# awikner/SPEEDY-ML-1

Hardware: AMD Instinct MI355X
Metric: hybrid timesteps/sec, T30L8 + 1152x6k-node reservoirs; 1/2/4/8-GPU scaling (higher is better)
Workload: dtype f64

## Files before the change

### include/speedy_ml.h

```cpp
#ifndef SPEEDY_ML_H
#define SPEEDY_ML_H

#include <stddef.h>
#include <stdint.h>

#ifdef __cplusplus
extern "C" {
#endif

#define SML_OK 0
#define SML_ERR_ARG (-1)
#define SML_ERR_HIP (-2)
#define SML_ERR_NOMEM (-3)
#define SML_ERR_STATE (-4)
#define SML_ERR_IO (-5)
#define SML_ERR_FORMAT (-6)

#define SML_F32 1
#define SML_F64 2

#define SML_MX 31
#define SML_NX 32
#define SML_MX2 62
#define SML_IX 96
// ... 85 lines not shown
int sml_nc_read_region(const char *path, int64_t *dims, float *win, float *wout, int *rows, int *cols, float *vals,
                       float *mean, float *std);
int sml_nc_write_region(const char *path, int n, int ninp, int nout, int ncs_plus_n, int k, const float *win,
                        const float *wout, const int *rows, const int *cols, const float *vals, const float *mean,
                        const float *std);

typedef struct sml_dynamics sml_dynamics;

int sml_dyn_create(double radius, sml_dynamics **out);
int sml_dyn_destroy(sml_dynamics *d);
int sml_dyn_impint(sml_dynamics *d, double dt, double alph);
int sml_dyn_set_forcing(sml_dynamics *d, const double *phis, const double *tcorh, const double *qcorh);
int sml_dyn_set_state(sml_dynamics *d, const double *vor, const double *div, const double *t, const double *ps,
                      const double *tr);
int sml_dyn_get_state(sml_dynamics *d, double *vor, double *div, double *t, double *ps, double *tr);
int sml_dyn_get_phi(sml_dynamics *d, double *phi);
int sml_dyn_get_tendencies(sml_dynamics *d, double *tend);
int sml_dyn_state_device(sml_dynamics *d, double **d_state, double **d_phys);
int sml_dyn_step(sml_dynamics *d, int j1, int j2, double dt, double alph, double rob, double wil,
                 const double *d_phys, void *stream);
int sml_dyn_leapfrog(sml_dynamics *d, int nsteps, double dt, double alph, double rob, double wil,
                     const double *d_phys, void *stream);
int sml_dyn_window(sml_dynamics *d, int nleap, double delt, double alph, double rob, double wil, void *stream);
int sml_dyn_from_grid(sml_dynamics *d, const double *d_grid4d, const double *d_logp, double *d_minmax,
                      void *stream);
int sml_dyn_to_grid(sml_dynamics *d, double *d_grid4d, double *d_logp, void *stream);
int sml_dyn_is_safe(const double *minmax);
int sml_dyn_run_model(sml_dynamics *d, const double *d_grid4d, const double *d_logp, int nleap, double delt,
                      double alph, double rob, double wil, double *d_fc4d, double *d_fc2d, void *stream);
int sml_dyn_last_safe(sml_dynamics *d, int *safe, double *minmax);
int sml_dyn_set_check_cus(sml_dynamics *d, int first_cu, int num_cus);
int sml_dyn_set_check_timeout(sml_dynamics *d, int64_t microseconds);
int sml_dyn_set_fused(sml_dynamics *d, int fused);
int sml_dyn_check_stream(const sml_dynamics *d, void **stream);
int sml_dyn_from_grid_host(sml_dynamics *d, const double *grid4d, const double *logp, double *minmax, int *safe);
int sml_dyn_to_grid_host(sml_dynamics *d, double *grid4d, double *logp);
int sml_dyn_step_host(sml_dynamics *d, int j1, int j2, double dt, double alph, double rob, double wil,
                      const double *phys);

int sml_dyn_set_physics(sml_dynamics *d, const double *bc);
int sml_dyn_set_hybrid_sst(sml_dynamics *d, const double *d_sst_grid, double sst_bias, void *stream);
int sml_dyn_set_sea_ice(sml_dynamics *d, const double *sice, const double *tice);
int sml_dyn_get_sea_ice(sml_dynamics *d, double *sice, double *tice);
int sml_dyn_get_physics(sml_dynamics *d, double *bc);
int sml_dyn_get_forcing(sml_dynamics *d, double *phis, double *tcorh, double *qcorh);
int sml_dyn_set_surface(sml_dynamics *d, const double *surface);
int sml_dyn_set_climatology(sml_dynamics *d, const double *clim);
int sml_dyn_fordate(sml_dynamics *d, int iyear, int imonth, int iday, void *stream);
int sml_dyn_fordate_ex(sml_dynamics *d, int iyear, int imonth, int iday, int force, void *stream);
int sml_dyn_fordate_count(const sml_dynamics *d, int *count);
int sml_dyn_set_clock(sml_dynamics *d, int istep, int lradsw);
int sml_dyn_get_clock(const sml_dynamics *d, int *istep, int *lradsw);
int sml_dyn_set_rad_state(sml_dynamics *d, const double *rad);
int sml_dyn_get_rad_state(sml_dynamics *d, double *rad);
int sml_dyn_phypar(sml_dynamics *d, const double *d_ug1, const double *d_vg1, const double *d_tg1,
                   const double *d_qg1, const double *d_phig1, const double *d_pslg1, int lradsw, double *d_tend,
                   void *stream);
int sml_dyn_phypar_host(sml_dynamics *d, const double *ug1, const double *vg1, const double *tg1, const double *qg1,
                        const double *phig1, const double *pslg1, int lradsw, double *tend);
int sml_dyn_sol_oz(const sml_dynamics *d, double tyear, double *fields5);
int sml_phys_sflset(const double *phi0, double *forog);

typedef struct sml_train sml_train;
int sml_train_create(int nlocal, const int *naug, int nout, sml_train **out);
int sml_train_destroy(sml_train *t);
int sml_train_reset(sml_train *t, void *stream);
// ... 88 lines not shown
```

### speedy-ml-1_amd/csrc/sml_dynamics.hip

```cpp
#include <hip/hip_runtime.h>

#include <cmath>
#include <cstddef>
#include <cstdlib>
#include <cstring>
#include <new>
#include <vector>

#include "sml_dynamics_tables.hpp"
#include "sml_fft.hpp"
#include "sml_fft_wa96.hpp"
#include "sml_physics.hpp"
#include "sml_physics_pair.hpp"
#include "sml_spectral_internal.hpp"
#include "sml_timeline.hpp"

SML_TL_DEFINE(dynamics)

using namespace sml;

namespace {

constexpr int kSF = kMX2 * kNX;
constexpr int kGF = kIX * kIL;
// ... 52 lines not shown
    unsigned chk_count = 0;
    bool chk_counted = false;
    double *h_mm = nullptr;
    hipEvent_t ev_mm = nullptr;
    bool mm_issued = false;
    const double *mm_last = nullptr;
    bool impint_done = false;
    PhysTables ptab;
    PhysTables *d_ptab = nullptr;
    double *d_pbc = nullptr, *d_rad = nullptr, *d_pio = nullptr;
    bool phys_on = false;
    double *d_sst_cpl = nullptr, *d_sice = nullptr, *d_tice = nullptr;
    const double *hyb_sst = nullptr;
    double hyb_bias = 0.0;
    double *d_surf = nullptr, *d_clim = nullptr, *d_ford = nullptr;
    bool surf_on = false, clim_on = false;
    long long ford_gen = 1, ford_done = 0;
    int ford_date[2] = {0, 0};
    int ford_count = 0;
    bool fused = true;
    bool nograph = false;
    bool lradsw = true;
    int istep = 1;
    hipStream_t cap_stream = nullptr;
    struct Replay {
        hipGraphExec_t exec = nullptr;
        double key[4] = {0, 0, 0, 0};
        const double *phys = nullptr;
        const DynTables *tab = nullptr;
        bool phys_on = false;
    } replay[2];
    struct WindowReplay {
        hipGraphExec_t exec = nullptr;
        double key[8] = {0, 0, 0, 0, 0, 0, 0, 0};
        DynTables *tab[3] = {nullptr, nullptr, nullptr};
        bool has_exit = false;
        const void *exit_key[16] = {};
    };
    static constexpr int kReplayWays = 4;
    WindowReplay wreplay[4][kReplayWays];
    int wreplay_next[4] = {0, 0, 0, 0};
    uint64_t *exit_store = nullptr;
    uint64_t exit_store_value = 0;
    uint64_t *d_xa = nullptr;
    bool entry_graph = true;
    bool serialized = false;
    uint64_t *d_go = nullptr;
    uint64_t go_count = 0;
    const uint64_t *go_src_next = nullptr;
    uint64_t *go_dst_next = nullptr;
    double *io_exit = nullptr;
};

namespace {

__device__ inline void uvspec_at(const double *vor, const double *div, const DynTables *T, int m, int n, double *uc,
                                 double *vc) {
    const double ux = T->uvdx[n][m];
    double zp[2], zc[2];
    zp[1] = ux * vor[ci(0, m, n)];
    zp[0] = -ux * vor[ci(1, m, n)];
    zc[1] = ux * div[ci(0, m, n)];
    zc[0] = -ux * div[ci(1, m, n)];
#pragma unroll
    for (int p = 0; p < 2; ++p) {
        double a, b;
        if (n == 0) {
            a = zc[p] - T->uvdyp[0][m] * vor[ci(p, m, 1)];
            b = zp[p] + T->uvdyp[0][m] * div[ci(p, m, 1)];
        } else if (n == kNX - 1) {
            a = T->uvdym[n][m] * vor[ci(p, m, kNTRUN1 - 1)];
            b = -T->uvdym[n][m] * div[ci(p, m, kNTRUN1 - 1)];
        } else {
            b = -T->uvdym[n][m] * div[ci(p, m, n - 1)] + T->uvdyp[n][m] * div[ci(p, m, n + 1)] + zp[p];
            a = T->uvdym[n][m] * vor[ci(p, m, n - 1)] - T->uvdyp[n][m] * vor[ci(p, m, n + 1)] + zc[p];
        }
        uc[ci(p, m, n)] = a;
        vc[ci(p, m, n)] = b;
// ... 1264 lines not shown
    if (mn >= kMN) return;
    const int k = blockIdx.y;
    const int m = mn % kMX, n = mn / kMX;
    const double trf = T->trfilt[n][m];
#pragma unroll
    for (int p = 0; p < 2; ++p) {
        const int c = ci(p, m, n);
        double vo, dv;
        vds_at(S + (size_t)k * kSF, S + (size_t)(kKX + k) * kSF, T, m, n, p, &vo, &dv);
        st[kOffVor + (size_t)k * kSF + c] = vo * trf;
        st[kOffDiv + (size_t)k * kSF + c] = dv * trf;
        st[kOffT + (size_t)k * kSF + c] = S[(size_t)(2 * kKX + k) * kSF + c] * trf;
        st[kOffTr + (size_t)k * kSF + c] = S[(size_t)(3 * kKX + k) * kSF + c] * trf;
        if (k == 0) st[kOffPs + c] = S[(size_t)(4 * kKX) * kSF + c] * trf;
    }
}

__global__ void k_io_prep(const double *__restrict__ st, double *__restrict__ sin_, const DynTables *__restrict__ T) {
    const int mn = blockIdx.x * blockDim.x + threadIdx.x;
    if (mn >= kMN) return;
    const int k = blockIdx.y;
    const int m = mn % kMX, n = mn / kMX;
    const double *vor = st + kOffVor + (size_t)k * kSF, *div = st + kOffDiv + (size_t)k * kSF;
    uvspec_at(vor, div, T, m, n, sin_ + (size_t)k * kSF, sin_ + (size_t)(kKX + k) * kSF);
#pragma unroll
    for (int p = 0; p < 2; ++p) {
        const int c = ci(p, m, n);
        sin_[(size_t)(2 * kKX + k) * kSF + c] = st[kOffT + (size_t)k * kSF + c];
        sin_[(size_t)(3 * kKX + k) * kSF + c] = st[kOffTr + (size_t)k * kSF + c];
        if (k == 0) sin_[(size_t)(4 * kKX) * kSF + c] = st[kOffPs + c];
    }
}

__global__ __launch_bounds__(kSpecThreads) void k_io_entry(const double *__restrict__ vio,
                                                           const double *__restrict__ pfl,
                                                           const double *__restrict__ wt, double *__restrict__ state,
                                                           double *__restrict__ sm, double *__restrict__ chk,
                                                           const double *__restrict__ phis,
                                                           const double *__restrict__ tabm,
                                                           const double *__restrict__ pinv, double *__restrict__ varm,
                                                           int n1, int nin, uint64_t *__restrict__ xa, uint64_t xa0,
                                                           uint64_t xa1) {
    SML_TL_SCOPE(sml::tl::kIoEntry);
    if (xa && blockIdx.x == 0 && threadIdx.x == 0) {
        xa[0] = xa0;
        xa[1] = xa1;
    }
    __shared__ double S[kNIo * kCW];
    __shared__ double Sst[kSM];
    __shared__ double In[kNInvMax * kCW];
    __shared__ double Fm[kCW];
    constexpr int RT = (kTabMDoubles / 2 + kSpecThreads - 1) / kSpecThreads;
    __shared__ double V[2 * RT * kSpecThreads];
    const int m = blockIdx.x, tid = threadIdx.x;
    const int wave = tid >> 6, l = tid & 63, r = l & 15, kk = l >> 4;
    constexpr int kSI = kSM / kSpecThreads;
    static_assert(kSM % kSpecThreads == 0 && kSI == 10, "slice staging: ten rows of the block");
    double s2[kSI / 2];
#pragma unroll
    for (int q = 1; q < kSI; q += 2) {
        const int cc = tid % kCW, k = tid / kCW, var = q / 2;
        const int c = ci(cc & 1, m, cc >> 1);
        double v = 0.0;
        if (var < 4) {
            const size_t off = var == 0 ? kOffVor : var == 1 ? kOffDiv : var == 2 ? kOffT : kOffTr;
            v = state[off + ((size_t)kKX + k) * kSF + c];
        } else if (k == 0) {
            v = state[kOffPs + (size_t)kSF + c];
        }
        s2[q / 2] = v;
    }
    const double phis_m = tid < kCW ? phis[ci(tid & 1, m, tid >> 1)] : 0.0;
    static_assert(2 * RT * kSpecThreads - kTabMDoubles <= kTabMPad, "TabM staging");
    double2 rt[RT];
    {
        const double2 *t = reinterpret_cast<const double2 *>(tabm + (size_t)m * kTabMDoubles) + tid;
#pragma unroll
        for (int q = 0; q < RT; ++q) rt[q] = t[q * kSpecThreads];
    }
    const bool spw = wave < (kNIo + 7) / 8;
    const int f0 = wave * 8, fa = f0 + (r >> 1);
    const bool ok = spw && fa < kNIo;
    double vn[kIY / 4], vs[kIY / 4], wv[kIY / 4], bS[kIY / 4], bD[kIY / 4];
    if (spw) {
        const double *vr = vio + (size_t)(ok ? fa : 0) * kVarmField + 2 * m + (r & 1);
        const double2 *pl = reinterpret_cast<const double2 *>(pfl) + (size_t)m * (kIY / 4) * 64 + l;
#pragma unroll
        for (int s = 0; s < kIY / 4; ++s) {
            const int j = 4 * s + kk;
            vn[s] = vr[(kIL - 1 - j) * kMX2];
            vs[s] = vr[j * kMX2];
            wv[s] = wt[j];
            const double2 b = pl[s * 64];
            bS[s] = b.x;
            bD[s] = b.y;
        }
    }
    const GridyB gb = gridy_operands(pinv, m);
    __builtin_amdgcn_sched_barrier(0);
#pragma unroll
    for (int q = 0; q < RT; ++q) reinterpret_cast<double2 *>(V)[tid + q * kSpecThreads] = rt[q];
#pragma unroll
    for (int q = 1; q < kSI; q += 2) Sst[tid + kSpecThreads * q] = s2[q / 2];
    if (tid < kCW) Fm[tid] = phis_m;
    if (spw) {
        d4 accS = {0, 0, 0, 0}, accD = accS;
#pragma unroll
        for (int s = 0; s < kIY / 4; ++s) {
            double aS = 0.0, aD = 0.0;
            if (ok) {
                aS = (vn[s] + vs[s]) * wv[s];
                aD = (vn[s] - vs[s]) * wv[s];
            }
            accS = MFMA64(aS, bS[s], accS);
            accD = MFMA64(aD, bD[s], accD);
        }
#pragma unroll
        for (int q = 0; q < 4; ++q) {
            const int row = kk + 4 * q;
            const int f = f0 + (row >> 1);
            if (f >= kNIo) continue;
            S[f * kCW + 2 * (2 * r) + (row & 1)] = accS[q];
            S[f * kCW + 2 * (2 * r + 1) + (row & 1)] = accD[q];
        }
    }
    __syncthreads();
    const LTab tb{reinterpret_cast<const TabM *>(V)};
    const int cc = tid & (kCW - 1), k = tid / kCW, n = cc >> 1, p = cc & 1, c = ci(p, m, n);
    {
        auto fl = [&](int f) { return [=](int pp, int nn) { return S[f * kCW + 2 * nn + pp]; }; };
        const double trf = tb.trfilt_n(n);
        double vo, dv;
        vds_gen(fl(k), fl(kKX + k), tb, n, p, &vo, &dv);
        const double v0 = vo * trf, v1 = dv * trf, v2 = S[(2 * kKX + k) * kCW + cc] * trf,
                     v3 = S[(3 * kKX + k) * kCW + cc] * trf;
        Sst[smi(0, 1, k, cc)] = v0;
        Sst[smi(1, 1, k, cc)] = v1;
        Sst[smi(2, 1, k, cc)] = v2;
        Sst[smi(3, 1, k, cc)] = v3;
        state[kOffVor + (size_t)k * kSF + c] = v0;
        state[kOffDiv + (size_t)k * kSF + c] = v1;
        state[kOffT + (size_t)k * kSF + c] = v2;
        state[kOffTr + (size_t)k * kSF + c] = v3;
        if (k == 0) {
            const double v4 = S[(4 * kKX) * kCW + cc] * trf;
            Sst[smi(4, 1, 0, cc)] = v4;
            state[kOffPs + c] = v4;
        } else {
            Sst[smi(4, 1, k, cc)] = 0.0;
        }
    }
    __syncthreads();
    {
        double a, b;
        uvspec_sel(Sst, tb, 1, k, n, p, &a, &b);
        chk[(size_t)k * kSF + c] = a;
        chk[(size_t)(kKX + k) * kSF + c] = b;
        chk[(size_t)(2 * kKX + k) * kSF + c] = Sst[smi(2, 1, k, cc)];
        chk[(size_t)(3 * kKX + k) * kSF + c] = Sst[smi(3, 1, k, cc)];
        if (k == 0) chk[(size_t)(4 * kKX) * kSF + c] = Sst[smi(4, 1, 0, cc)];
    }
    {
        static_assert(kSM / 2 % kSpecThreads == 0, "slice rows");
        constexpr int R = kSM / 2 / kSpecThreads;
        double2 *dst = reinterpret_cast<double2 *>(sm + (size_t)m * kSM) + tid;
        const double2 *src = reinterpret_cast<const double2 *>(Sst) + tid;
        double2 v[R];
#pragma unroll
        for (int q = 0; q < R; ++q) v[q] = src[q * kSpecThreads];
#pragma unroll
        for (int q = 0; q < R; ++q) dst[q * kSpecThreads] = v[q];
    }
    inv_inputs(Sst, In, Fm, tb, m, 1, n1, nin);
    __syncthreads();
    gridy_m(In, gb, varm, m, nin);
}

__device__ inline double nmin(double a, double b) { return (a != a || b != b) ? __builtin_nan("") : (b < a ? b : a); }
__device__ inline double nmax(double a, double b) { return (a != a || b != b) ? __builtin_nan("") : (b > a ? b : a); }

__global__ void k_flag_store_value(uint64_t *flag, uint64_t v) {
    SML_TL_SCOPE(sml::tl::kExitStore);
    if (threadIdx.x == 0) __hip_atomic_store(flag, v, __ATOMIC_RELAXED, __HIP_MEMORY_SCOPE_AGENT);
}
__global__ void k_set_xa(uint64_t *xa, uint64_t v0, uint64_t v1, uint64_t v2, uint64_t v3) {
    if (threadIdx.x == 0) {
        xa[0] = v0;
        xa[1] = v1;
        xa[2] = v2;
        xa[3] = v3;
    }
}

__global__ void k_check_go(const uint64_t *go, uint64_t want, unsigned *late, unsigned late_value, long long timeout) {
    if (threadIdx.x != 0) return;
    const long long t0 = wall_clock64();
    while (__hip_atomic_load(go, __ATOMIC_RELAXED, __HIP_MEMORY_SCOPE_AGENT) < want) {
        __builtin_amdgcn_s_sleep(2);
        if (wall_clock64() - t0 > timeout) {
            __hip_atomic_store(late, late_value, __ATOMIC_RELAXED, __HIP_MEMORY_SCOPE_SYSTEM);
            break;
        }
    }
    __builtin_amdgcn_fence(__ATOMIC_ACQUIRE, "agent");
}

__global__ void k_flag_store(uint64_t *flag, const uint64_t *xa) {
    SML_TL_SCOPE(sml::tl::kExitStore);
// ... 421 lines not shown
                              void *stream) {
    SML_REQUIRE(d && nleap >= 0 && delt > 0.0, "bad argument");
    return window_impl(d, nleap, delt, alph, rob, wil, stream, false);
}

namespace {
int window_impl(sml_dynamics *d, int nleap, double delt, double alph, double rob, double wil, void *stream,
                bool prepared, const ExitSpec *exit) {
    const double dts[3] = {0.5 * delt, delt, 2.0 * delt};
    DynTables *tab[3];
    for (int i = 0; i < 3; ++i) {
        if (int rc = sml_dyn_impint(d, dts[i], alph)) return rc;
        tab[i] = d->d_tab;
    }
    const bool entry = d->lradsw;
    if (d->nograph) {
        hipStream_t st = (hipStream_t)stream;
        d->d_tab = tab[0];
        d->io_exit = prepared ? d->d_varm : nullptr;
        int rc = launch_step(d, 1, 1, dts[0], alph, rob, wil, nullptr, entry, st, prepared, 2);
        d->d_tab = tab[1];
        if (!rc) rc = launch_step(d, 1, 2, dts[1], alph, rob, wil, nullptr, entry, st, true, nleap > 0 ? 2 : 0);
        d->d_tab = tab[2];
        for (int i = 0; i < nleap && !rc; ++i)
            rc = launch_step(d, 2, 2, dts[2], alph, rob, wil, nullptr, (1 + i) % kNstrad == 1, st, true,
                             i + 1 < nleap ? 2 : 0);
        d->io_exit = nullptr;
        if (rc) return rc;
        d->istep = 1 + nleap;
        if (nleap > 0) d->lradsw = (nleap % kNstrad == 1);
        return SML_OK;
    }
    const int cls = (entry ? 1 : 0) + (prepared ? 2 : 0);
    const double key[8] = {(double)nleap, delt,  alph, rob, wil, d->phys_on ? 1.0 : 0.0, d->fused ? 1.0 : 0.0,
                           prepared ? 2.0 : 1.0};
    const void *exit_key[16] = {};
    if (exit) {
        const EntrySpec *en = exit->entry;
        const void *k[16] = {exit->varm,   exit->fc4,     exit->fc2,    exit->ex.mm,
                             exit->ex.in4, exit->ex.inlp, exit->ex.cnt, (const void *)(intptr_t)exit->ex.timeout,
                             exit->store,  en ? (const void *)1 : nullptr,
                             en ? en->w.flag : nullptr, en ? en->w.late : nullptr, en ? en->w.sig : nullptr,
                             en ? (const void *)(intptr_t)en->w.timeout : nullptr, en ? en->w.vptr : nullptr,
                             en ? en->go : nullptr};
        std::memcpy(exit_key, k, sizeof k);
    }
    auto same = [&](const sml_dynamics::WindowReplay &w) {
        return w.exec && w.has_exit == (exit != nullptr) &&
               (!exit || std::memcmp(exit_key, w.exit_key, sizeof exit_key) == 0) &&
               std::memcmp(key, w.key, sizeof key) == 0 && std::memcmp(tab, w.tab, sizeof tab) == 0;
    };
    sml_dynamics::WindowReplay *hit = nullptr;
    for (auto &w : d->wreplay[cls])
        if (same(w)) hit = &w;
    if (!hit) {
        hit = &d->wreplay[cls][d->wreplay_next[cls]];
        d->wreplay_next[cls] = (d->wreplay_next[cls] + 1) % sml_dynamics::kReplayWays;
    }
    sml_dynamics::WindowReplay &r = *hit;
    if (!same(r)) {
        if (r.exec) {
            SML_HIP(hipGraphExecDestroy(r.exec));
            r.exec = nullptr;
        }
        r.has_exit = false;
        if (!d->cap_stream) SML_HIP(hipStreamCreateWithFlags(&d->cap_stream, hipStreamNonBlocking));
        hipGraph_t g = nullptr;
        SML_HIP(hipStreamBeginCapture(d->cap_stream, hipStreamCaptureModeThreadLocal));
// ... 8 lines not shown
        d->io_exit = prepared ? d->d_varm : nullptr;
        if (!rc) rc = launch_step(d, 1, 1, dts[0], alph, rob, wil, nullptr, entry, d->cap_stream, prepared, 2);
        d->go_src_next = nullptr;
        d->go_dst_next = nullptr;
        d->d_tab = tab[1];
        if (!rc) rc = launch_step(d, 1, 2, dts[1], alph, rob, wil, nullptr, entry, d->cap_stream, true, nleap > 0 ? 2 : 0);
        d->d_tab = tab[2];
        for (int i = 0; i < nleap && !rc; ++i)
            rc = launch_step(d, 2, 2, dts[2], alph, rob, wil, nullptr, (1 + i) % kNstrad == 1, d->cap_stream, true,
                             i + 1 < nleap ? 2 : 0);
        if (!rc && exit) {
            rc = spectral_gridx_run_model_exit(d->sp, exit->varm, exit->fc4, exit->fc2, kNIoWind, exit->ex,
                                               d->cap_stream);
            if (!rc && exit->store) {
                hipLaunchKernelGGL(k_flag_store, dim3(1), dim3(64), 0, d->cap_stream, exit->store, exit->ex.xa);
                if (hipGetLastError() != hipSuccess) rc = fail(SML_ERR_HIP, "k_flag_store capture");
            }
        }
        hipError_t e = hipStreamEndCapture(d->cap_stream, &g);
        d->io_exit = nullptr;
        if (rc) {
            if (g) (void)hipGraphDestroy(g);
            return rc;
        }
        if (e != hipSuccess) return fail(SML_ERR_HIP, "sml_dyn_window capture: %s", hipGetErrorString(e));
        e = hipGraphInstantiate(&r.exec, g, nullptr, nullptr, 0);
        if (e != hipSuccess) {
            (void)hipGraphDestroy(g);
            r.exec = nullptr;
            return fail(SML_ERR_HIP, "sml_dyn_window instantiate: %s", hipGetErrorString(e));
        }
        (void)hipGraphDestroy(g);
        r.has_exit = exit != nullptr;
        std::memcpy(r.exit_key, exit_key, sizeof exit_key);
        std::memcpy(r.key, key, sizeof key);
        std::memcpy(r.tab, tab, sizeof tab);
    }
    SML_HIP(hipGraphLaunch(r.exec, (hipStream_t)stream));
    d->d_tab = tab[2];
    d->istep = 1 + nleap;
    if (nleap > 0) d->lradsw = (nleap % kNstrad == 1);
    return SML_OK;
}
}

extern "C" int sml_dyn_set_clock(sml_dynamics *d, int istep, int lradsw) {
    SML_REQUIRE(d, "null context");
    d->istep = istep;
    d->lradsw = lradsw != 0;
    return SML_OK;
}

extern "C" int sml_dyn_get_clock(const sml_dynamics *d, int *istep, int *lradsw) {
    SML_REQUIRE(d, "null context");
    if (istep) *istep = d->istep;
    if (lradsw) *lradsw = d->lradsw ? 1 : 0;
    return SML_OK;
}

namespace {
__global__ void k_hybrid_sst(const double *__restrict__ cpl, const double *__restrict__ hyb,
                             const double *__restrict__ sice, const double *__restrict__ tice, double bias,
                             double *__restrict__ sst_am) {
#pragma clang fp contract(off)
    const int p = blockIdx.x * blockDim.x + threadIdx.x;
    if (p >= kNGP) return;
    double s = cpl[p];
    if (hyb) {
        const double diff = s - hyb[p];
        if (diff < 6.0) s = hyb[p];
        s = s + bias;
// ... 320 lines not shown
    if (int rc = spectral_gridx_range(d->sp, cv, cg, kNIo, 0, kNIoWind, cst)) return rc;
    double *mm = d_minmax ? d_minmax : d->d_minmax;
    const bool counted = cst != st && !d_minmax;
    hipLaunchKernelGGL(k_io_minmax, dim3(4), dim3(1024), 0, cst, cg, mm, counted ? d->d_chk_cnt : nullptr,
                       go ? d->d_chk_late : nullptr, 4u * (d->chk_count + 1));
    SML_HIP(hipGetLastError());
    if (counted) ++d->chk_count;
    d->chk_counted = counted;
    d->mm_last = mm;
    d->mm_issued = false;
    if (cst != st) {
        if (!d->h_mm) {
            SML_HIP(hipHostMalloc((void **)&d->h_mm, 8 * sizeof(double), hipHostMallocDefault));
            SML_HIP(hipEventCreateWithFlags(&d->ev_mm, hipEventDisableTiming));
        }
        SML_HIP(hipMemcpyAsync(d->h_mm, mm, 8 * sizeof(double), hipMemcpyDeviceToHost, cst));
        SML_HIP(hipEventRecord(d->ev_mm, cst));
        d->mm_issued = true;
        SML_HIP(hipEventRecord(d->ev_chk, cst));
        d->chk_pending = true;
        if (d_minmax) {
            SML_HIP(hipStreamWaitEvent(st, d->ev_chk, 0));
            d->chk_pending = false;
        }
    }
    return SML_OK;
}

int launch_entry(sml_dynamics *d, const double *d_grid4d, const double *d_logp, HopWait w, hipStream_t st,
                 uint64_t *xa, uint64_t xa0, uint64_t xa1) {
    if (int rc = spectral_specx_io(d->sp, d_grid4d, d_logp, d->d_vfm, kNIoWind, st, w)) return rc;
    const SpectralDev sd = spectral_dev(d->sp);
    const bool phys = d->phys_on;
    hipLaunchKernelGGL(k_io_entry, dim3(kMX), dim3(kSpecThreads), 0, st, d->d_vfm, d->d_pfl, sd.wt, d->d_state,
                       sm_buf(d, 0), d->d_chk, d->d_phis,
                       d->d_tabm + (size_t)(d->d_tab - d->d_tabs) * kMX * kTabMDoubles, sd.pinv, d->d_varm,
                       phys ? kNInv1P : kNInv1, phys ? kNInvP : kNInv, xa, xa0, xa1);
    SML_HIP(hipGetLastError());
    return SML_OK;
}
}

extern "C" int sml_dyn_from_grid(sml_dynamics *d, const double *d_grid4d, const double *d_logp, double *d_minmax,
                                 void *stream) {
    SML_REQUIRE(d && d_grid4d && d_logp, "null argument");
    hipStream_t st = (hipStream_t)stream;
    const DynTables *T = d->d_tab;
    if (d->chk_pending) {
        SML_HIP(hipStreamWaitEvent(st, d->ev_chk, 0));
        d->chk_pending = false;
    }
    HopWait w = d->entry_wait;
    w.sig = d->entry_sig;
    d->entry_wait = HopWait{};
    d->entry_sig = nullptr;
    if (int rc = spectral_specx_io(d->sp, d_grid4d, d_logp, d->d_varm, kNIoWind, st, w)) return rc;
    if (int rc = spectral_specy(d->sp, d->d_varm, d->d_sfwd, kNIo, st)) return rc;
    hipLaunchKernelGGL(k_io_combine, dim3((kMN + 127) / 128, kKX), dim3(128), 0, st, d->d_sfwd, d->d_state, T);
    SML_HIP(hipGetLastError());
    hipLaunchKernelGGL(k_io_prep, dim3((kMN + 127) / 128, kKX), dim3(128), 0, st, d->d_state, d->d_chk, T);
    SML_HIP(hipGetLastError());
    return launch_io_check(d, st, d_minmax);
}

extern "C" int sml_dyn_to_grid(sml_dynamics *d, double *d_grid4d, double *d_logp, void *stream) {
    SML_REQUIRE(d && d_grid4d && d_logp, "null argument");
    hipStream_t st = (hipStream_t)stream;
    hipLaunchKernelGGL(k_io_prep, dim3((kMN + 127) / 128, kKX), dim3(128), 0, st, d->d_state, d->d_specin, d->d_tab);
    SML_HIP(hipGetLastError());
    if (int rc = spectral_gridy(d->sp, d->d_specin, d->d_varm, kNIo, st)) return rc;
    return spectral_gridx_io(d->sp, d->d_varm, d_grid4d, d_logp, kNIoWind, st);
// ... 141 lines not shown
    if (d->d_chk_late && d->chk_counted &&
        __atomic_load_n(d->d_chk_late, __ATOMIC_ACQUIRE) == 4u * d->chk_count)
        *safe = 0;
    if (minmax) std::memcpy(minmax, mm, sizeof mm);
    return SML_OK;
}

int sml::dyn_run_model_wait(sml_dynamics *d, const uint64_t *flag, uint64_t value, unsigned *late,
                            long long timeout) {
    SML_REQUIRE(d && flag && late, "null argument");
    d->entry_wait = HopWait{flag, value, late};
    d->entry_wait.timeout = timeout;
    return SML_OK;
}

int sml::dyn_set_check_timeout(sml_dynamics *d, long long timeout) {
    SML_REQUIRE(d && timeout >= 0, "bad argument");
    d->chk_timeout = timeout;
    return SML_OK;
}

extern "C" int sml_dyn_set_check_timeout(sml_dynamics *d, int64_t microseconds) {
    SML_REQUIRE(d && microseconds >= 0, "bad argument");
    if (d->chk_stream) SML_HIP(hipStreamSynchronize(d->chk_stream));
    return sml::dyn_set_check_timeout(d, (long long)std::min<int64_t>(microseconds, INT64_MAX / 100) * 100);
}

extern "C" int sml_dyn_set_fused(sml_dynamics *d, int fused) {
    SML_REQUIRE(d, "null context");
    d->fused = fused != 0;
    return SML_OK;
}

extern "C" int sml_dyn_check_stream(const sml_dynamics *d, void **stream) {
    SML_REQUIRE(d && stream, "null argument");
    *stream = d->chk_stream;
    return SML_OK;
}

int sml::dyn_check_event(sml_dynamics *d, void **ev) {
    SML_REQUIRE(d && ev, "null argument");
    *ev = d->chk_stream ? (void *)d->ev_chk : nullptr;
    return SML_OK;
}

int sml::dyn_run_model_entry_signal(sml_dynamics *d, uint64_t *counter, int *adds) {
    SML_REQUIRE(d && counter && adds, "null argument");
    d->entry_sig = counter;
    *adds = spectral_specx_io_blocks();
    return SML_OK;
}

int sml::dyn_run_model_exit_store(sml_dynamics *d, uint64_t *flag, uint64_t value) {
    SML_REQUIRE(d, "null argument");
    d->exit_store = flag;
    d->exit_store_value = value;
    return SML_OK;
}

int sml::dyn_check_late(sml_dynamics *d) {
    if (!d || !d->d_chk_late) return SML_OK;
    if (__atomic_load_n(d->d_chk_late, __ATOMIC_ACQUIRE)) {
        __atomic_store_n(d->d_chk_late, 0u, __ATOMIC_RELEASE);
        return fail(SML_ERR_STATE, "run_model's exit did not receive its safety check in time (window taken as unsafe)");
    }
    return SML_OK;
// ... 54 lines not shown
```

### speedy-ml-1_amd/speedy_ml_amd/_lib.py

```python
from __future__ import annotations

import ctypes
import os
import subprocess

PKG_ROOT = os.path.dirname(os.path.dirname(os.path.abspath(__file__)))
LIB_PATH = os.environ.get("SML_LIB") or os.path.join(PKG_ROOT, "lib", "libspeedyml.so")
CSRC = os.path.join(PKG_ROOT, "csrc")

SML_OK = 0
SML_F32 = 1
SML_F64 = 2

EXPORTED = (
    "sml_last_error", "sml_abi_version",
    "sml_spectral_create", "sml_spectral_destroy", "sml_spectral_tables",
    "sml_grid_batched", "sml_spec_batched", "sml_gridy_batched", "sml_gridx_batched",
    "sml_specx_batched", "sml_specy_batched", "sml_vdspec_batched", "sml_uvspec_batched",
    "sml_grid_host", "sml_spec_host",
    "sml_res_create", "sml_res_destroy", "sml_res_ninp", "sml_res_feedback_offsets",
    "sml_res_load_region_f32", "sml_res_load_region_f64", "sml_res_set_state", "sml_res_get_state",
    "sml_res_step", "sml_res_step_begin", "sml_res_step_finish", "sml_res_step_finish_grid", "sml_res_step_finish_assemble", "sml_res_step_host", "sml_res_synchronize",
    "sml_res_footprint", "sml_res_enable_timing", "sml_res_kernel_times", "sml_res_set_read_waves",
    "sml_res_set_begin_mode", "sml_res_begin_fused",
    "sml_exchange_assemble",
    "sml_res_tile_inputs", "sml_res_tile_feedback", "sml_res_tile_local_model",
    "sml_nc_read_region", "sml_nc_write_region",
    "sml_dyn_create", "sml_dyn_destroy", "sml_dyn_impint", "sml_dyn_set_forcing", "sml_dyn_set_state",
    "sml_dyn_get_state", "sml_dyn_get_phi", "sml_dyn_get_tendencies", "sml_dyn_state_device",
    "sml_dyn_step", "sml_dyn_step_host", "sml_dyn_leapfrog", "sml_dyn_window", "sml_dyn_from_grid", "sml_dyn_to_grid",
    "sml_dyn_is_safe", "sml_dyn_from_grid_host", "sml_dyn_to_grid_host",
    "sml_dyn_set_physics", "sml_dyn_set_clock", "sml_dyn_get_clock", "sml_dyn_set_rad_state",
    "sml_dyn_get_rad_state", "sml_dyn_phypar", "sml_dyn_phypar_host", "sml_dyn_sol_oz", "sml_phys_sflset",
    "sml_train_create", "sml_train_destroy", "sml_train_reset", "sml_train_accumulate", "sml_train_solve",
    "sml_train_npad", "sml_train_get_gram", "sml_probe_mfma_f64",
    "sml_stream_create_cu_range", "sml_stream_destroy",
    "sml_dyn_run_model", "sml_dyn_last_safe", "sml_dyn_set_check_cus", "sml_res_info",
    "sml_comm_unique_id", "sml_comm_create", "sml_comm_create_file", "sml_comm_destroy", "sml_comm_rank",
    "sml_comm_allgather",
    "sml_hybrid_create", "sml_hybrid_destroy", "sml_hybrid_set_buffers", "sml_hybrid_set_tisr",
    "sml_hybrid_streams", "sml_hybrid_cus", "sml_hybrid_start", "sml_hybrid_predict", "sml_hybrid_advance", "sml_hybrid_step",
    "sml_hybrid_run_speedy", "sml_hybrid_sync",
    "sml_device_alloc", "sml_device_free", "sml_copy_to_device", "sml_copy_to_host", "sml_region_geometry",
    "sml_processor_decomposition", "sml_hybrid_set_tisr_table", "sml_tisr_date_index", "sml_res_tile_tisr_field",
    "sml_res_create_generic", "sml_res_step_slab", "sml_res_start_prediction",
    "sml_comm_create_local", "sml_exchange_plan", "sml_hybrid_advance_slabs", "sml_hybrid_set_hop_mode",
    "sml_hybrid_hop_mode", "sml_calendar_delta_hour", "sml_hybrid_set_feb29", "sml_hybrid_get_feb29",
    "sml_res_mean_std", "sml_res_set_outvec_ld", "sml_hybrid_set_slab", "sml_hybrid_start_slab",
    "sml_hybrid_exchange_width", "sml_hybrid_slab_buffers", "sml_dyn_set_hybrid_sst", "sml_dyn_set_sea_ice",
    "sml_hybrid_set_pipelined", "sml_res_step_cancel", "sml_res_step_begun", "sml_hybrid_set_force_exchange",
    "sml_hybrid_exchanges", "sml_hybrid_set_chain", "sml_hybrid_chain", "sml_hybrid_exchange_stream",
    "sml_res_set_update_cus", "sml_res_update_balanced", "sml_probe_mfma_f64_clock", "sml_res_ell_layout",
    "sml_dyn_get_sea_ice", "sml_dyn_get_physics", "sml_dyn_get_forcing", "sml_dyn_set_surface",
    "sml_dyn_set_climatology", "sml_dyn_fordate", "sml_dyn_fordate_ex", "sml_dyn_fordate_count",
    "sml_hybrid_set_calendar", "sml_hybrid_window_date", "sml_hybrid_set_hop_timeout",
    "sml_dyn_set_check_timeout", "sml_dyn_check_stream", "sml_dyn_set_fused", "sml_res_set_reference_paths",
    "sml_train_set_panel",
)

SML_HOP_AUTO, SML_HOP_WAIT_VALUE, SML_HOP_EVENTS, SML_HOP_KERNEL = 0, 1, 2, 3
SML_CHAIN_AUTO, SML_CHAIN_TWO_STREAMS, SML_CHAIN_SPEEDY = 0, 1, 2
SML_RES_PATH_CSR, SML_RES_PATH_PER_REGION, SML_RES_PATH_UNGROUPED_FINISH = 1, 2, 4


class SmlError(RuntimeError):
    pass


_lib = None


def build(jobs: int = 8) -> str:
    subprocess.run(["make", "-s", "-C", CSRC, f"-j{jobs}"], check=True)
    return LIB_PATH


def lib() -> ctypes.CDLL:
    global _lib
    if _lib is None:
        if not os.path.exists(LIB_PATH):
            raise SmlError(f"{LIB_PATH} is missing: build it with `make -C {CSRC}` "
                           "(or __graft_entry__.build()); there is no CPU fallback")
        L = ctypes.CDLL(LIB_PATH)
        _declare(L)
        _lib = L
    return _lib


def check(rc: int) -> None:
# ... 64 lines not shown
        "sml_dyn_step_host": [vp, i, i, d, d, d, d, vp],
        "sml_dyn_leapfrog": [vp, i, d, d, d, d, vp, vp],
        "sml_dyn_window": [vp, i, d, d, d, d, vp],
        "sml_dyn_from_grid": [vp, vp, vp, vp, vp],
        "sml_dyn_to_grid": [vp, vp, vp, vp],
        "sml_dyn_is_safe": [vp],
        "sml_dyn_from_grid_host": [vp, vp, vp, vp, ctypes.POINTER(ctypes.c_int)],
        "sml_dyn_to_grid_host": [vp, vp, vp],
        "sml_dyn_set_physics": [vp, vp],
        "sml_dyn_set_clock": [vp, i, i],
        "sml_dyn_get_clock": [vp, ctypes.POINTER(ctypes.c_int), ctypes.POINTER(ctypes.c_int)],
        "sml_dyn_set_rad_state": [vp, vp],
        "sml_dyn_get_rad_state": [vp, vp],
        "sml_dyn_phypar": [vp, vp, vp, vp, vp, vp, vp, i, vp, vp],
        "sml_dyn_phypar_host": [vp, vp, vp, vp, vp, vp, vp, i, vp],
        "sml_dyn_sol_oz": [vp, d, vp],
        "sml_phys_sflset": [vp, vp],
        "sml_train_create": [i, vp, i, pp],
        "sml_train_destroy": [vp],
        "sml_train_reset": [vp, vp],
        "sml_train_accumulate": [vp, vp, vp, i, vp],
        "sml_train_solve": [vp, i, d, d, i, d, vp, vp, vp],
        "sml_train_npad": [vp, ctypes.POINTER(ctypes.c_int)],
        "sml_train_get_gram": [vp, i, vp, vp],
        "sml_probe_mfma_f64": [i, ctypes.POINTER(ctypes.c_double)],
        "sml_stream_create_cu_range": [i, i, pp],
        "sml_stream_destroy": [vp],
        "sml_dyn_run_model": [vp, vp, vp, i, d, d, d, d, vp, vp, vp],
        "sml_dyn_last_safe": [vp, ip, vp],
        "sml_dyn_set_check_cus": [vp, i, i],
        "sml_dyn_set_check_timeout": [vp, ctypes.c_int64],
        "sml_dyn_check_stream": [vp, pp],
        "sml_dyn_set_fused": [vp, i],
        "sml_res_set_reference_paths": [vp, i],
        "sml_train_set_panel": [vp, i],
        "sml_res_info": [vp, ip, ip, ip, ip, vp],
        "sml_comm_unique_id": [vp],
        "sml_comm_create": [i, i, vp, pp],
        "sml_comm_create_file": [i, i, ctypes.c_char_p, i, pp],
        "sml_comm_destroy": [vp],
        "sml_comm_rank": [vp, ip, ip],
        "sml_comm_allgather": [vp, vp, vp, ctypes.c_int64, vp],
        "sml_hybrid_create": [vp, vp, vp, i, d, d, d, d, i, i, pp],
        "sml_hybrid_destroy": [vp],
        "sml_hybrid_set_buffers": [vp, vp, vp, vp, vp, vp, vp, vp, vp, vp],
        "sml_hybrid_set_tisr": [vp, vp],
        "sml_hybrid_streams": [vp, pp, pp],
        "sml_hybrid_cus": [vp, ip, ip],
        "sml_hybrid_start": [vp, vp, vp, vp, vp, vp],
        "sml_hybrid_predict": [vp],
        "sml_hybrid_advance": [vp, vp],
        "sml_hybrid_step": [vp],
        "sml_hybrid_run_speedy": [vp, ip],
        "sml_hybrid_sync": [vp],
        "sml_device_alloc": [ctypes.c_int64, pp],
        "sml_device_free": [vp],
        "sml_copy_to_device": [vp, vp, ctypes.c_int64],
        "sml_copy_to_host": [vp, vp, ctypes.c_int64],
        "sml_region_geometry": [i, i, ip],
        "sml_processor_decomposition": [i, i, i, ip, ip],
        "sml_hybrid_set_tisr_table": [vp, vp, i, i, ctypes.c_int64, i],
        "sml_tisr_date_index": [i, ctypes.c_int64, ip, ip],
        "sml_res_tile_tisr_field": [vp, vp, vp, vp],
        "sml_res_create_generic": [i, i, vp, vp, vp, vp, i, i, vp, i, d, pp],
        "sml_res_step_slab": [vp, vp, vp, vp, vp, vp],
        "sml_res_start_prediction": [vp, vp, i, ctypes.c_int64, vp, vp],
# ... 63 lines not shown
```

### speedy-ml-1_amd/speedy_ml_amd/dynamics.py

```python
from __future__ import annotations

import ctypes

import numpy as np

from ._lib import check, lib, ptr, stream_ptr

EARTH_RADIUS = 6.371e6
KX, NX, MX = 8, 32, 31
FIELDS = ("vor", "div", "t", "tr", "ps")
NSTEPS = 96
NGP = 96 * 48
PHYS_BC = ("fmask1", "phis0", "stl_am", "sst_am", "soilw_am", "alb_l", "alb_s", "albsfc", "snowc",
           "fsol", "ozone", "ozupp", "zenit", "stratz", "forog")
SURFACE = ("fmask_l", "fmask_s", "alb0")
CLIMATOLOGY = ("stl12", "snowd12", "soilw12", "sst12", "sice12")
RAD_SIZE = (4 * KX + 2 + KX + 1) * NGP
DELT = 86400.0 / NSTEPS
ROB, WIL, ALPH = 0.05, 0.53, 0.5


def _c128(a, shape):
    a = np.ascontiguousarray(a, dtype=np.complex128)
    if a.shape != shape:
        raise ValueError(f"expected shape {shape}, got {a.shape}")
    return a


class Dynamics:
    def __init__(self, radius: float = EARTH_RADIUS):
        h = ctypes.c_void_p()
        check(lib().sml_dyn_create(radius, ctypes.byref(h)))
        self._h = h
        self._dtal = None

    def close(self):
        if self._h:
            lib().sml_dyn_destroy(self._h)
            self._h = None

    __del__ = close

    def set_fused(self, fused: bool):
        check(lib().sml_dyn_set_fused(self._h, int(bool(fused))))

    def impint(self, dt: float, alph: float = ALPH):
        check(lib().sml_dyn_impint(self._h, dt, alph))
        self._dtal = (dt, alph)

    def set_forcing(self, phis=None, tcorh=None, qcorh=None):
        args = [None if a is None else _c128(a, (NX, MX)) for a in (phis, tcorh, qcorh)]
        check(lib().sml_dyn_set_forcing(self._h, *[ptr(a) for a in args]))

    def set_state(self, state):
        a = {f: _c128(state[f], (2, KX, NX, MX) if f != "ps" else (2, NX, MX)) for f in FIELDS}
        check(lib().sml_dyn_set_state(self._h, ptr(a["vor"]), ptr(a["div"]), ptr(a["t"]), ptr(a["ps"]),
                                      ptr(a["tr"])))

    def get_state(self):
        out = {f: np.zeros((2, KX, NX, MX) if f != "ps" else (2, NX, MX), np.complex128) for f in FIELDS}
        check(lib().sml_dyn_get_state(self._h, ptr(out["vor"]), ptr(out["div"]), ptr(out["t"]), ptr(out["ps"]),
                                      ptr(out["tr"])))
        return out

    def get_phi(self):
        phi = np.zeros((KX, NX, MX), np.complex128)
        check(lib().sml_dyn_get_phi(self._h, ptr(phi)))
        return phi

    def get_tendencies(self):
        tend = np.zeros((4 * KX + 1, NX, MX), np.complex128)
        check(lib().sml_dyn_get_tendencies(self._h, ptr(tend)))
        return tend

    def device_buffers(self):
        s, p = ctypes.c_void_p(), ctypes.c_void_p()
        check(lib().sml_dyn_state_device(self._h, ctypes.byref(s), ctypes.byref(p)))
        return s.value, p.value
# ... 176 lines not shown
```

Before: 1168.

## Split io entry kernel across two blocks per wavenumber for gridy work

Templates the k_io_entry kernel on a split factor and launches by default with kSpecSplit blocks per zonal wavenumber m, matching k_st_spec's layout. Each block redoes the spectral staging. Only the lead block writes state and slice outputs and only the last block writes check outputs. The gridy_m latitude tiles are divided between the blocks, each staging its pinv slice in shared memory. This aims to cut the entry kernel's latency by using more CUs, at the cost of duplicated staging work and extra shared memory. The split factor is also added to the graph replay key.

Result: no change. 1171, median of 6 (+0.2%).

```diff
diff --git a/include/speedy_ml.h b/include/speedy_ml.h
--- a/include/speedy_ml.h
+++ b/include/speedy_ml.h
@@ -141,6 +141,8 @@
 int sml_dyn_set_check_cus(sml_dynamics *d, int first_cu, int num_cus);
 int sml_dyn_set_check_timeout(sml_dynamics *d, int64_t microseconds);
 int sml_dyn_set_fused(sml_dynamics *d, int fused);
+int sml_dyn_set_entry_split(sml_dynamics *d, int blocks_per_m);
+int sml_dyn_entry_split(const sml_dynamics *d, int *requested, int *last);
 int sml_dyn_check_stream(const sml_dynamics *d, void **stream);
 int sml_dyn_from_grid_host(sml_dynamics *d, const double *grid4d, const double *logp, double *minmax, int *safe);
 int sml_dyn_to_grid_host(sml_dynamics *d, double *grid4d, double *logp);
diff --git a/speedy-ml-1_amd/csrc/sml_dynamics.hip b/speedy-ml-1_amd/csrc/sml_dynamics.hip
--- a/speedy-ml-1_amd/csrc/sml_dynamics.hip
+++ b/speedy-ml-1_amd/csrc/sml_dynamics.hip
@@ -108,10 +108,11 @@
     } replay[2];
     struct WindowReplay {
         hipGraphExec_t exec = nullptr;
-        double key[8] = {0, 0, 0, 0, 0, 0, 0, 0};
+        double key[9] = {0, 0, 0, 0, 0, 0, 0, 0, 0};
         DynTables *tab[3] = {nullptr, nullptr, nullptr};
         bool has_exit = false;
         const void *exit_key[16] = {};
+        int entry_form = 0;
     };
     static constexpr int kReplayWays = 4;
     WindowReplay wreplay[4][kReplayWays];
@@ -120,6 +121,8 @@
     uint64_t exit_store_value = 0;
     uint64_t *d_xa = nullptr;
     bool entry_graph = true;
+    int entry_split = 2;
+    int entry_ran = 0;
     bool serialized = false;
     uint64_t *d_go = nullptr;
     uint64_t go_count = 0;
@@ -1450,6 +1453,7 @@
     }
 }
 
+template <int kSplit>
 __global__ __launch_bounds__(kSpecThreads) void k_io_entry(const double *__restrict__ vio,
                                                            const double *__restrict__ pfl,
                                                            const double *__restrict__ wt, double *__restrict__ state,
@@ -1469,8 +1473,14 @@
     __shared__ double In[kNInvMax * kCW];
     __shared__ double Fm[kCW];
     constexpr int RT = (kTabMDoubles / 2 + kSpecThreads - 1) / kSpecThreads;
-    __shared__ double V[2 * RT * kSpecThreads];
-    const int m = blockIdx.x, tid = threadIdx.x;
+    constexpr int kPinvM = kNX * 32, kVPinv = 2 * RT * kSpecThreads;
+    static_assert(kSplit == 1 || kSplit == kSpecSplit, "k_io_entry: one block per m or k_st_spec's split");
+    static_assert(kPinvM == 2 * kSpecThreads, "pinv slice staging: one double2 per thread");
+    __shared__ double V[kVPinv + (kSplit > 1 ? kPinvM : 0)];
+    const int m = kSplit > 1 ? blockIdx.x % kSpecStride : blockIdx.x, half = kSplit > 1 ? blockIdx.x / kSpecStride : 0;
+    if (m >= kMX) return;
+    const bool lead = half == 0, checks = half == kSplit - 1;
+    const int tid = threadIdx.x;
     const int wave = tid >> 6, l = tid & 63, r = l & 15, kk = l >> 4;
     constexpr int kSI = kSM / kSpecThreads;
     static_assert(kSM % kSpecThreads == 0 && kSI == 10, "slice staging: ten rows of the block");
@@ -1514,13 +1524,19 @@
             bD[s] = b.y;
         }
     }
-    const GridyB gb = gridy_operands(pinv, m);
+    GridyB gb;
+    double2 rp = {0.0, 0.0};
+    if constexpr (kSplit > 1)
+        rp = reinterpret_cast<const double2 *>(pinv + (size_t)m * kPinvM)[tid];
+    else
+        gb = gridy_operands(pinv, m);
     __builtin_amdgcn_sched_barrier(0);
 #pragma unroll
     for (int q = 0; q < RT; ++q) reinterpret_cast<double2 *>(V)[tid + q * kSpecThreads] = rt[q];
 #pragma unroll
     for (int q = 1; q < kSI; q += 2) Sst[tid + kSpecThreads * q] = s2[q / 2];
     if (tid < kCW) Fm[tid] = phis_m;
+    if constexpr (kSplit > 1) reinterpret_cast<double2 *>(V + kVPinv)[tid] = rp;
     if (spw) {
         d4 accS = {0, 0, 0, 0}, accD = accS;
 #pragma unroll
@@ -1556,20 +1572,22 @@
         Sst[smi(1, 1, k, cc)] = v1;
         Sst[smi(2, 1, k, cc)] = v2;
         Sst[smi(3, 1, k, cc)] = v3;
-        state[kOffVor + (size_t)k * kSF + c] = v0;
-        state[kOffDiv + (size_t)k * kSF + c] = v1;
-        state[kOffT + (size_t)k * kSF + c] = v2;
-        state[kOffTr + (size_t)k * kSF + c] = v3;
+        if (lead) {
+            state[kOffVor + (size_t)k * kSF + c] = v0;
+            state[kOffDiv + (size_t)k * kSF + c] = v1;
+            state[kOffT + (size_t)k * kSF + c] = v2;
+            state[kOffTr + (size_t)k * kSF + c] = v3;
+        }
         if (k == 0) {
             const double v4 = S[(4 * kKX) * kCW + cc] * trf;
             Sst[smi(4, 1, 0, cc)] = v4;
-            state[kOffPs + c] = v4;
+            if (lead) state[kOffPs + c] = v4;
         } else {
             Sst[smi(4, 1, k, cc)] = 0.0;
         }
     }
     __syncthreads();
-    {
+    if (checks) {
         double a, b;
         uvspec_sel(Sst, tb, 1, k, n, p, &a, &b);
         chk[(size_t)k * kSF + c] = a;
@@ -1578,7 +1596,7 @@
         chk[(size_t)(3 * kKX + k) * kSF + c] = Sst[smi(3, 1, k, cc)];
         if (k == 0) chk[(size_t)(4 * kKX) * kSF + c] = Sst[smi(4, 1, 0, cc)];
     }
-    {
+    if (lead) {
         static_assert(kSM / 2 % kSpecThreads == 0, "slice rows");
         constexpr int R = kSM / 2 / kSpecThreads;
         double2 *dst = reinterpret_cast<double2 *>(sm + (size_t)m * kSM) + tid;
@@ -1591,7 +1609,12 @@
     }
     inv_inputs(Sst, In, Fm, tb, m, 1, n1, nin);
     __syncthreads();
-    gridy_m(In, gb, varm, m, nin);
+    if constexpr (kSplit > 1) {
+        const int nt = (nin + 7) / 8, per = (nt + kSplit - 1) / kSplit;
+        gridy_m(In, gridy_operands_slice(V + kVPinv), varm, m, nin, half * per, min(nt, (half + 1) * per));
+    } else {
+        gridy_m(In, gb, varm, m, nin);
+    }
 }
 
 __device__ inline double nmin(double a, double b) { return (a != a || b != b) ? __builtin_nan("") : (b < a ? b : a); }
@@ -2079,8 +2102,8 @@
         return SML_OK;
     }
     const int cls = (entry ? 1 : 0) + (prepared ? 2 : 0);
-    const double key[8] = {(double)nleap, delt,  alph, rob, wil, d->phys_on ? 1.0 : 0.0, d->fused ? 1.0 : 0.0,
-                           prepared ? 2.0 : 1.0};
+    const double key[9] = {(double)nleap, delt,  alph, rob, wil, d->phys_on ? 1.0 : 0.0, d->fused ? 1.0 : 0.0,
+                           prepared ? 2.0 : 1.0, exit && exit->entry ? (double)d->entry_split : 0.0};
     const void *exit_key[16] = {};
     if (exit) {
         const EntrySpec *en = exit->entry;
@@ -2155,11 +2178,13 @@
         }
         (void)hipGraphDestroy(g);
         r.has_exit = exit != nullptr;
+        r.entry_form = exit && exit->entry ? d->entry_ran : 0;
         std::memcpy(r.exit_key, exit_key, sizeof exit_key);
         std::memcpy(r.key, key, sizeof key);
         std::memcpy(r.tab, tab, sizeof tab);
     }
     SML_HIP(hipGraphLaunch(r.exec, (hipStream_t)stream));
+    if (r.entry_form) d->entry_ran = r.entry_form;
     d->d_tab = tab[2];
     d->istep = 1 + nleap;
     if (nleap > 0) d->lradsw = (nleap % kNstrad == 1);
@@ -2546,11 +2571,17 @@
     if (int rc = spectral_specx_io(d->sp, d_grid4d, d_logp, d->d_vfm, kNIoWind, st, w)) return rc;
     const SpectralDev sd = spectral_dev(d->sp);
     const bool phys = d->phys_on;
-    hipLaunchKernelGGL(k_io_entry, dim3(kMX), dim3(kSpecThreads), 0, st, d->d_vfm, d->d_pfl, sd.wt, d->d_state,
-                       sm_buf(d, 0), d->d_chk, d->d_phis,
-                       d->d_tabm + (size_t)(d->d_tab - d->d_tabs) * kMX * kTabMDoubles, sd.pinv, d->d_varm,
-                       phys ? kNInv1P : kNInv1, phys ? kNInvP : kNInv, xa, xa0, xa1);
+    const double *tabm = d->d_tabm + (size_t)(d->d_tab - d->d_tabs) * kMX * kTabMDoubles;
+    const int n1 = phys ? kNInv1P : kNInv1, nin = phys ? kNInvP : kNInv;
+    if (d->entry_split == kSpecSplit)
+        hipLaunchKernelGGL(k_io_entry<kSpecSplit>, dim3(kSpecStride * kSpecSplit), dim3(kSpecThreads), 0, st, d->d_vfm,
+                           d->d_pfl, sd.wt, d->d_state, sm_buf(d, 0), d->d_chk, d->d_phis, tabm, sd.pinv, d->d_varm, n1,
+                           nin, xa, xa0, xa1);
+    else
+        hipLaunchKernelGGL(k_io_entry<1>, dim3(kMX), dim3(kSpecThreads), 0, st, d->d_vfm, d->d_pfl, sd.wt, d->d_state,
+                           sm_buf(d, 0), d->d_chk, d->d_phis, tabm, sd.pinv, d->d_varm, n1, nin, xa, xa0, xa1);
     SML_HIP(hipGetLastError());
+    d->entry_ran = d->entry_split;
     return SML_OK;
 }
 }
@@ -2758,6 +2789,19 @@
     return SML_OK;
 }
 
+extern "C" int sml_dyn_set_entry_split(sml_dynamics *d, int blocks_per_m) {
+    SML_REQUIRE(d && (blocks_per_m == 1 || blocks_per_m == kSpecSplit), "blocks_per_m is 1 or 2");
+    d->entry_split = blocks_per_m;
+    return SML_OK;
+}
+
+extern "C" int sml_dyn_entry_split(const sml_dynamics *d, int *requested, int *last) {
+    SML_REQUIRE(d, "null context");
+    if (requested) *requested = d->entry_split;
+    if (last) *last = d->entry_ran;
+    return SML_OK;
+}
+
 extern "C" int sml_dyn_check_stream(const sml_dynamics *d, void **stream) {
     SML_REQUIRE(d && stream, "null argument");
     *stream = d->chk_stream;
diff --git a/speedy-ml-1_amd/speedy_ml_amd/_lib.py b/speedy-ml-1_amd/speedy_ml_amd/_lib.py
--- a/speedy-ml-1_amd/speedy_ml_amd/_lib.py
+++ b/speedy-ml-1_amd/speedy_ml_amd/_lib.py
@@ -55,6 +55,7 @@
     "sml_dyn_set_climatology", "sml_dyn_fordate", "sml_dyn_fordate_ex", "sml_dyn_fordate_count",
     "sml_hybrid_set_calendar", "sml_hybrid_window_date", "sml_hybrid_set_hop_timeout",
     "sml_dyn_set_check_timeout", "sml_dyn_check_stream", "sml_dyn_set_fused", "sml_res_set_reference_paths",
+    "sml_dyn_set_entry_split", "sml_dyn_entry_split",
     "sml_train_set_panel",
 )
 
@@ -185,6 +186,8 @@
         "sml_dyn_set_check_timeout": [vp, ctypes.c_int64],
         "sml_dyn_check_stream": [vp, pp],
         "sml_dyn_set_fused": [vp, i],
+        "sml_dyn_set_entry_split": [vp, i],
+        "sml_dyn_entry_split": [vp, ip, ip],
         "sml_res_set_reference_paths": [vp, i],
         "sml_train_set_panel": [vp, i],
         "sml_res_info": [vp, ip, ip, ip, ip, vp],
diff --git a/speedy-ml-1_amd/speedy_ml_amd/dynamics.py b/speedy-ml-1_amd/speedy_ml_amd/dynamics.py
--- a/speedy-ml-1_amd/speedy_ml_amd/dynamics.py
+++ b/speedy-ml-1_amd/speedy_ml_amd/dynamics.py
@@ -44,6 +44,14 @@
     def set_fused(self, fused: bool):
         check(lib().sml_dyn_set_fused(self._h, int(bool(fused))))
 
+    def set_entry_split(self, blocks_per_m: int):
+        check(lib().sml_dyn_set_entry_split(self._h, int(blocks_per_m)))
+
+    def entry_split(self):
+        a, b = ctypes.c_int(), ctypes.c_int()
+        check(lib().sml_dyn_entry_split(self._h, ctypes.byref(a), ctypes.byref(b)))
+        return a.value, b.value
+
     def impint(self, dt: float, alph: float = ALPH):
         check(lib().sml_dyn_impint(self._h, dt, alph))
         self._dtal = (dt, alph)
```
